# Quantco/tabmat

Measured on AMD Instinct MI355X. Metric: SplitMatrix.sandwich GFLOP/s + effective HBM GB/s, 10M×1k mixed, higher is better.
Workload: dtype f64; 1 GPU; SplitMatrix.sandwich: dense128 + csr512@5% + cats(256,96,32), 10000000 rows/GPU, p=1024, float64 (BASELINE configs[3]); rows_per_gpu=10000000, p=1024, launch=eager, collective=none

## Files before the change

tabmat_amd/csrc/syrk_co.hip:

```cpp
#include <algorithm>

#include "common.hpp"

namespace tmh {

constexpr int CO_RS = 12;
constexpr int CO_W = 128;
constexpr int CO_LDW = CO_W + 16;
constexpr int CO_CPI = 64;
constexpr int CO_ITEM_ROWS = CO_CPI * CO_RS;
constexpr int CO_T = 36;
constexpr int CO_NWAVES = 4;
constexpr int CO_THREADS = CO_NWAVES * 64;
constexpr int CO_CHUNK = CO_RS * CO_LDW;
constexpr size_t CO_LDS = sizeof(double) * (size_t)(2 * CO_CHUNK + 2 * CO_RS) + 32 + sizeof(double) * CO_W;
constexpr size_t CO_LDS_TV = CO_LDS + sizeof(double) * 2 * CO_RS;

typedef double co_acc_t __attribute__((ext_vector_type(4)));
typedef double co_vec2 __attribute__((ext_vector_type(2)));

constexpr int co_tri_row(int t) {
    int r = 0;
    while ((r + 1) * (r + 2) / 2 <= t) ++r;
    return r;
// ... 151 lines not shown
            for (int b = 0; b < 8; ++b) xa[b] = dv0 * xb0[b];
            cs0 += xa[2 * WID];
            cs1 += xa[2 * WID + 1];
            if constexpr (TV) {
                cv0 = __builtin_fma(vv0, xb0[2 * WID], cv0);
                cv1 = __builtin_fma(vv0, xb0[2 * WID + 1], cv1);
            }
            co_mfma_set<WID, 0>(xa, xb0, acc);
            __syncthreads();
            if (pending) { idNext = *slot; pending = false; }
            id_c = id_c1;
            id_c1 = id_c2;
            buf ^= 1;
        }
        double *dst = part + (int64_t)blockIdx.x * (CO_T * 256);
#pragma unroll
        for (int s = 0; s < 9; ++s) {
            const int t = WID + s * CO_NWAVES;
#pragma unroll
            for (int r = 0; r < 4; ++r)
                dst[t * 256 + ((lane >> 4) + 4 * r) * 16 + (lane & 15)] = acc[s][r];
        }
        cs0 += __shfl_xor(cs0, 16, 64);
        cs0 += __shfl_xor(cs0, 32, 64);
        cs1 += __shfl_xor(cs1, 16, 64);
        cs1 += __shfl_xor(cs1, 32, 64);
        if (lane < 16) {
            double *cd = cpart + (int64_t)blockIdx.x * CO_W;
            cd[32 * WID + 2 * lane] = cs0;
            cd[32 * WID + 2 * lane + 1] = cs1;
        }
        if constexpr (TV) {
            cv0 += __shfl_xor(cv0, 16, 64);
            cv0 += __shfl_xor(cv0, 32, 64);
            cv1 += __shfl_xor(cv1, 16, 64);
            cv1 += __shfl_xor(cv1, 32, 64);
            if (lane < 16) {
                double *vd = vpart + (int64_t)blockIdx.x * CO_W;
                vd[32 * WID + 2 * lane] = cv0;
                vd[32 * WID + 2 * lane + 1] = cv1;
            }
        }
    };
    if (wave == 0) run(std::integral_constant<int, 0>{});
    else if (wave == 1) run(std::integral_constant<int, 1>{});
    else if (wave == 2) run(std::integral_constant<int, 2>{});
    else run(std::integral_constant<int, 3>{});
    if (tid == 0) wg_log_end(log, t_begin, WG_SYRK_CO);
}

__global__ __launch_bounds__(1024) void syrk_co_finish_kernel(const double *__restrict__ part,
                                                              int nblk, int n_cols,
                                                              double *__restrict__ out, int64_t ldo,
                                                              const unsigned *__restrict__ only_if) {
    if (only_if != nullptr && *only_if == 0) return;
    __shared__ double red[16][64];
    const int e = blockIdx.y * 64 + threadIdx.x, s = threadIdx.y, t = blockIdx.x;
    double a = 0.0;
    for (int b = s; b < nblk; b += 16) a += part[((int64_t)b * CO_T + t) * 256 + e];
    red[s][threadIdx.x] = a;
    __syncthreads();
    if (s == 0) {
        double v = 0.0;
#pragma unroll
        for (int w = 0; w < 16; w += 4)
            v += (red[w][threadIdx.x] + red[w + 1][threadIdx.x]) +
                 (red[w + 2][threadIdx.x] + red[w + 3][threadIdx.x]);
        int bi = 0;
        while ((bi + 1) * (bi + 2) / 2 <= t) ++bi;
        const int bj = t - bi * (bi + 1) / 2;
        const int ci = co_actual_col(16 * bi + (e >> 4)), cj = co_actual_col(16 * bj + (e & 15));
        if (ci < n_cols && cj < n_cols && (bi != bj || (e >> 4) >= (e & 15))) {
            out[(int64_t)ci * ldo + cj] = v;
            if (ci != cj) out[(int64_t)cj * ldo + ci] = v;
        }
    }
}

__global__ __launch_bounds__(CO_W) void syrk_co_colsum_kernel(const double *__restrict__ cpart,
                                                              int nblk, int n_cols,
                                                              double *__restrict__ colsum,
                                                              const unsigned *__restrict__ only_if) {
    if (only_if != nullptr && *only_if == 0u) return;
    const int c = threadIdx.x;
    double a = 0.0;
    for (int b = 0; b < nblk; ++b) a += cpart[(int64_t)b * CO_W + c];
    if (c < n_cols) colsum[c] = a;
}

size_t syrk_co_ws_bytes() {
    const size_t grid = (size_t)std::max<int64_t>(1, tune("co_grid", 3 * NUM_CU));
    return 256 + sizeof(double) * grid * (CO_T * 256 + 2 * CO_W);
}

static int run_syrk_co_impl(const double *X, int64_t ldx, int64_t n, int64_t m, const double *d, double *out,
                            int64_t ldo, double *colsum, const unsigned *only_if, void *ws_given,
                            hipStream_t st, const double *center, const double *v, double *xtv) {
    TM_REQUIRE((v == nullptr) == (xtv == nullptr), "v and xtv go together");
    TM_REQUIRE(n >= 0 && m >= 0, "negative shape");
    TM_REQUIRE(m == 0 || syrk_co_ok(X, m),
               "the co-resident syrk takes a 16-byte aligned C-ordered block of <= 128 columns");
    if (m == 0) return TM_OK;
    if (n == 0) {
        TM_HIP(hipMemset2DAsync(out, sizeof(double) * (size_t)ldo, 0, sizeof(double) * (size_t)m, (size_t)m, st));
        if (colsum) TM_HIP(hipMemsetAsync(colsum, 0, sizeof(double) * (size_t)m, st));
        if (xtv) TM_HIP(hipMemsetAsync(xtv, 0, sizeof(double) * (size_t)m, st));
        return TM_OK;
    }
    const int64_t n_items64 = ceil_div(n, CO_ITEM_ROWS);
    TM_REQUIRE(n_items64 < (1ll << 31), "too many rows");
    const int n_items = (int)n_items64;
    const int grid = (int)std::min<int64_t>(n_items, tune("co_grid", 3 * NUM_CU));
    const size_t part_bytes = sizeof(double) * (size_t)grid * CO_T * 256;
    const size_t cpart_bytes = sizeof(double) * (size_t)grid * CO_W * (v ? 2 : 1);
    void *wsv = ws_given;
    if (wsv == nullptr) {
        int rc = get_workspace(256 + part_bytes + cpart_bytes, &wsv, st);
        if (rc) return rc;
    }
    unsigned *counter = reinterpret_cast<unsigned *>(wsv);
    double *part = reinterpret_cast<double *>(reinterpret_cast<char *>(wsv) + 256);
    double *cpart = part + (size_t)grid * CO_T * 256;
    double *vpart = v ? cpart + (size_t)grid * CO_W : nullptr;
    TM_HIP(hipMemsetAsync(counter, 0, 256, st));
    auto kern = v ? ((m & 1) ? (center ? &syrk_co_kernel<true, true, true> : &syrk_co_kernel<false, true, true>)
                             : (center ? &syrk_co_kernel<true, false, true> : &syrk_co_kernel<false, false, true>))
                  : ((m & 1) ? (center ? &syrk_co_kernel<true, true> : &syrk_co_kernel<false, true>)
                             : (center ? &syrk_co_kernel<true, false> : &syrk_co_kernel<false, false>));
    const size_t lds = v ? CO_LDS_TV : CO_LDS;
    TM_HIP(hipFuncSetAttribute(reinterpret_cast<const void *>(kern),
                               hipFuncAttributeMaxDynamicSharedMemorySize, (int)lds));
    prof_begin(st);
    hipLaunchKernelGGL(kern, dim3((unsigned)grid), dim3(CO_THREADS), lds, st, X, n, ldx,
                       (int)m, d, n_items, counter, part, cpart, wg_log_ptr(), only_if, center, v, vpart);
    prof_end(st);
    TM_LAUNCH_CHECK();
    hipLaunchKernelGGL(syrk_co_finish_kernel, dim3(CO_T, 4), dim3(64, 16), 0, st, part, grid, (int)m,
                       out, ldo, only_if);
    TM_LAUNCH_CHECK();
    if (colsum) {
        hipLaunchKernelGGL(syrk_co_colsum_kernel, dim3(1), dim3(CO_W), 0, st, cpart, grid, (int)m,
                           colsum, only_if);
        TM_LAUNCH_CHECK();
    }
    if (xtv) {
        hipLaunchKernelGGL(syrk_co_colsum_kernel, dim3(1), dim3(CO_W), 0, st, vpart, grid, (int)m,
                           xtv, only_if);
        TM_LAUNCH_CHECK();
    }
    return TM_OK;
}

int run_syrk_co(const double *X, int64_t n, int64_t m, const double *d, double *out, double *colsum,
                hipStream_t st, const double *center, const double *v, double *xtv) {
    return run_syrk_co_impl(X, m, n, m, d, out, m, colsum, nullptr, nullptr, st, center, v, xtv);
}

int run_syrk_co_flagged(const double *X, int64_t ldx, int64_t n, int64_t m, const double *d, double *out,
                        int64_t ldo, double *colsum, const unsigned *flag, void *ws, hipStream_t st,
                        const double *center, const double *v, double *xtv) {
    return run_syrk_co_impl(X, ldx, n, m, d, out, ldo, colsum, flag, ws, st, center, v, xtv);
}

}

using namespace tmh;

extern "C" {

int tm_dense_sandwich_co_f64(const double *X, int64_t n, int64_t m, const double *d, double *out,
                             double *colsum, void *stream) {
    return run_syrk_co(X, n, m, d, out, colsum, as_stream(stream));
}

int tm_dense_sandwich_co_centered_f64(const double *X, int64_t n, int64_t m, const double *d, const double *center,
                                      double *out, double *colsum, void *stream) {
    return run_syrk_co(X, n, m, d, out, colsum, as_stream(stream), center);
}

int tm_dense_sandwich_co_xtv_f64(const double *X, int64_t n, int64_t m, const double *d, const double *v,
                                 double *out, double *colsum, double *xtv, void *stream) {
    TM_REQUIRE(v != nullptr && xtv != nullptr, "v and xtv are required");
    return run_syrk_co(X, n, m, d, out, colsum, as_stream(stream), nullptr, v, xtv);
}

int tm_dense_sandwich_co_centered_xtv_f64(const double *X, int64_t n, int64_t m, const double *d, const double *v,
                                          const double *center, double *out, double *colsum, double *xtv,
                                          void *stream) {
    TM_REQUIRE(v != nullptr && xtv != nullptr, "v and xtv are required");
    return run_syrk_co(X, n, m, d, out, colsum, as_stream(stream), center, v, xtv);
}

}
```

tabmat_amd/csrc/syrk_i8.hip:

```cpp
#include <algorithm>
#include <cmath>

#include "common.hpp"

#if defined(I8_NO_SB)
#define I8_SB
#else
#define I8_SB __builtin_amdgcn_sched_barrier(0)
#endif
#if defined(I8_TRACE)
#define I8_STAMP(k)                                                                                     \
    do {                                                                                                \
        if (blockIdx.x == 0 && lane == 0 && trace_it >= 8 && trace_it < 12)                             \
            trace_buf[((trace_it - 8) * 4 + wave) * 8 + (k)] = __builtin_readcyclecounter();            \
    } while (0)
#else
#define I8_STAMP(k)
#endif
namespace tmh {

constexpr int I8_W = 128;
constexpr int I8_T = 36;
constexpr int I8_ND = 5;
constexpr int I8_WLO = 2;
constexpr int I8_NC = 2 * (I8_ND - 1) - I8_WLO + 1;
constexpr int I8_FBITS = 38;
constexpr int I8_RS = 64;
constexpr int I8_HS = 32;
constexpr int I8_WAVES = 4;
constexpr int I8_THREADS = I8_WAVES * 64;
constexpr int I8_PSTR = 64;
constexpr int I8_PLANE = I8_W * I8_PSTR;
constexpr int I8_PLANES = I8_ND * I8_PLANE;
constexpr int I8_RAWSTR = 1024 + 32;
constexpr int I8_RAWBUF = I8_HS * I8_RAWSTR;
#ifndef I8_DMA_AUX
#define I8_DMA_AUX 0
#endif
#ifndef I8_CPI_N
#define I8_CPI_N 32
#endif
constexpr int I8_CPI = I8_CPI_N;
constexpr int I8_ITEM_ROWS = I8_CPI * I8_RS;
constexpr size_t I8_LDS = (size_t)I8_PLANES + 3 * (size_t)I8_RAWBUF + 3 * I8_HS * sizeof(double) + 16;
static_assert(I8_LDS <= 160 * 1024, "planes + the ring of 3 half chunks fill the CU's LDS");

typedef int i8_v4 __attribute__((ext_vector_type(4)));

struct I8Info {
    unsigned dmax_bits_hi;
    unsigned dmax_bits_lo;
    unsigned flag;
    unsigned pad;
};

constexpr int i8_pair_find(int idx, bool want_s) {
    int k = 0;
    for (int w = I8_WLO; w <= 2 * (I8_ND - 1); ++w)
        for (int s = 0; s < I8_ND; ++s) {
            const int t = w - s;
            if (t < 0 || t >= I8_ND) continue;
            if (k == idx) return want_s ? s : t;
            ++k;
        }
    return -1;
}
constexpr int i8_pair_s(int idx) { return i8_pair_find(idx, true); }
constexpr int i8_pair_t(int idx) { return i8_pair_find(idx, false); }
constexpr int i8_count_pairs() {
    int k = 0;
    while (i8_pair_find(k, true) >= 0) ++k;
    return k;
}
constexpr int I8_NP = i8_count_pairs();
static_assert(I8_NP == 22, "the pair groups of the chunk loop are laid out for 22 pairs");

template <int WID>
struct I8Tiles {
    static constexpr int NB = 5;
    static constexpr int block(int l) {
        constexpr int B[4][5] = {{0, 1, 2, 3, 4}, {0, 1, 5, 6, 7}, {2, 3, 5, 6, 7}, {3, 4, 5, 6, 7}};
        return B[WID][l];
    }
    static constexpr int local(int b) {
        for (int l = 0; l < NB; ++l)
            if (block(l) == b) return l;
        return 0;
    }
    static constexpr int bi(int q) {
        constexpr int T[4][9] = {{1, 2, 3, 4, 2, 3, 4, 3, 4}, {5, 6, 7, 5, 6, 7, 6, 0, 1},
                                 {5, 6, 7, 5, 6, 7, 7, 2, 3}, {5, 6, 7, 4, 7, 4, 5, 6, 7}};
        return T[WID][q];
    }
    static constexpr int bj(int q) {
        constexpr int T[4][9] = {{0, 0, 0, 0, 1, 1, 1, 2, 2}, {0, 0, 0, 1, 1, 1, 5, 0, 1},
                                 {2, 2, 2, 3, 3, 3, 5, 2, 3}, {4, 4, 4, 3, 6, 4, 5, 6, 7}};
        return T[WID][q];
    }
    static constexpr int tile(int q) { return bi(q) * (bi(q) + 1) / 2 + bj(q); }
};

#if defined(__HIP_DEVICE_COMPILE__)
typedef __amdgpu_buffer_rsrc_t i8_rsrc_t;
__device__ __forceinline__ i8_rsrc_t i8_rsrc(const void *base, int64_t bytes) {
    const unsigned nb = bytes <= 0 ? 0u : (bytes > 0xFFFFFFFFll ? 0xFFFFFFFFu : (unsigned)bytes);
    return __builtin_amdgcn_make_buffer_rsrc(const_cast<void *>(base), 0, (int)nb, 0x00020000);
}
__device__ __forceinline__ void i8_dma16(i8_rsrc_t rs, void *lds, int voff) {
    __builtin_amdgcn_raw_ptr_buffer_load_lds(rs, (__attribute__((address_space(3))) void *)lds, 16, voff, 0, 0, I8_DMA_AUX);
}
__device__ __forceinline__ void i8_lds_barrier() { asm volatile("s_waitcnt lgkmcnt(0)\n\ts_barrier" ::: "memory"); }
__device__ __forceinline__ unsigned i8_perm(unsigned hi, unsigned lo, unsigned sel) {
    return __builtin_amdgcn_perm(hi, lo, sel);
}
#else
struct i8_rsrc_t {};
inline i8_rsrc_t i8_rsrc(const void *, int64_t) { return {}; }
inline void i8_dma16(i8_rsrc_t, void *, int) {}
inline void i8_lds_barrier() {}
inline unsigned i8_perm(unsigned, unsigned, unsigned) { return 0; }
#endif

__global__ __launch_bounds__(256) void i8_screen_kernel(const double *__restrict__ d, int64_t n, I8Info *info) {
    double mx = 0.0;
    bool bad = false;
    const int64_t stride = (int64_t)gridDim.x * blockDim.x;
    int64_t i = (int64_t)blockIdx.x * blockDim.x + threadIdx.x;
    for (; i + 3 * stride < n; i += 4 * stride) {
        const double v0 = d[i], v1 = d[i + stride], v2 = d[i + 2 * stride], v3 = d[i + 3 * stride];
        bad |= !(v0 >= 0.0) || !(v0 <= 1.7e308) || !(v1 >= 0.0) || !(v1 <= 1.7e308) ||
               !(v2 >= 0.0) || !(v2 <= 1.7e308) || !(v3 >= 0.0) || !(v3 <= 1.7e308);
        mx = fmax(fmax(mx, fmax(v0, v1)), fmax(v2, v3));
    }
    for (; i < n; i += stride) {
        const double v = d[i];
        bad |= !(v >= 0.0) || !(v <= 1.7e308);
        mx = fmax(mx, v);
    }
    for (int off = 32; off > 0; off >>= 1) {
        mx = fmax(mx, __shfl_down(mx, off, 64));
        bad |= (bool)__shfl_down((int)bad, off, 64);
    }
    __shared__ double wmx[4];
    __shared__ int wbad[4];
    if ((threadIdx.x & 63) == 0) {
        wmx[threadIdx.x >> 6] = mx;
        wbad[threadIdx.x >> 6] = (int)bad;
    }
    __syncthreads();
    if (threadIdx.x == 0) {
        mx = fmax(fmax(wmx[0], wmx[1]), fmax(wmx[2], wmx[3]));
        if (wbad[0] | wbad[1] | wbad[2] | wbad[3]) atomicOr(&info->flag, 1u);
        atomicMax(reinterpret_cast<unsigned long long *>(info), (unsigned long long)__double_as_longlong(mx > 0.0 ? mx : 0.0));
    }
}

__global__ void i8_scale_kernel(const double *__restrict__ colmax, int m, int64_t n_rows, I8Info *info,
                                double *__restrict__ sigma, double *__restrict__ rscale, int *history) {
    const int i = threadIdx.x;
    if (history != nullptr && i == 0) {
        const int calls = history[1]++;
        if (history[0] >= 3 && (calls & 31) != 0) atomicOr(&info->flag, 4u);
    }
    if (i >= I8_W) return;
    const double dmax = __longlong_as_double(*reinterpret_cast<const long long *>(info));
    if (history != nullptr && i < m && n_rows > 0) {
        const double prev = reinterpret_cast<const double *>(history + 4)[i];
        const double bound = fmin(64.0, 134217728.0 / (double)n_rows);
        if (prev > 0.0 && !(colmax[i] * colmax[i] * dmax <= bound * prev)) atomicOr(&info->flag, 4u);
    }
    __syncthreads();
    double s = 1.0, r = 1.0;
    if (i < m) {
        const double big = colmax[i] * sqrt(dmax);
        if (big > 0.0 && info->flag == 0) {
            int e;
            frexp(big, &e);
            s = ldexp(1.0, I8_FBITS - e);
            r = ldexp(1.0, e - I8_FBITS);
        }
    }
    sigma[i] = s;
    rscale[i] = r;
}

template <bool CSUM, bool CEN, bool TV = false>
__global__ __launch_bounds__(I8_THREADS) __attribute__((amdgpu_waves_per_eu(1, 1)))
void syrk_i8_kernel(const double *__restrict__ X, int64_t ldx, int64_t n, int64_t m, const double *__restrict__ d,
                    const double *__restrict__ sigma, const I8Info *__restrict__ info, int n_items,
                    unsigned *__restrict__ counter, double *__restrict__ part, double *__restrict__ colsum,
                    const double *__restrict__ center, const double *__restrict__ v = nullptr,
                    double *__restrict__ xtv = nullptr) {
    if (info->flag != 0) return;
    __shared__ __attribute__((aligned(16))) unsigned char planes[I8_PLANES];
    __shared__ __attribute__((aligned(16))) unsigned char raw[3 * I8_RAWBUF];
    __shared__ double dl[3 * I8_HS];
    __shared__ double vl[TV ? 3 * I8_HS : 1];
    __shared__ unsigned slot_mem[4];
    unsigned *slot = slot_mem;
#if defined(I8_TRACE)
    unsigned long long *trace_buf = reinterpret_cast<unsigned long long *>(reinterpret_cast<char *>(counter) - 256 + 2560);
    int trace_it = 0;
#endif

    const int tid = threadIdx.x;
    const int lane = tid & 63;
    const int wave = __builtin_amdgcn_readfirstlane(tid >> 6);
    const int cl = lane & 15, rq = lane >> 4;

    unsigned idL = blockIdx.x;
    int hL = 0;
    unsigned idNext;
    if (tid == 0) *slot = gridDim.x + atomicAdd(counter, 1u);
    __syncthreads();
    idNext = __builtin_amdgcn_readfirstlane(*slot);
    bool pending = false;

    using C0 = std::integral_constant<int, 0>;
    using C1 = std::integral_constant<int, 1>;
    double dreg = 0.0, vreg = 0.0;
    const int dma_voff = lane * 2 < m ? lane * 16 : 0x7ffffff0;
    auto issue_half = [&](int rb) -> unsigned {
        const unsigned id = idL;
        const int64_t tb = (int64_t)id * I8_ITEM_ROWS + (int64_t)hL * I8_HS;
        const int64_t left = min((n - tb) * ldx * 8, (int64_t)I8_HS * ldx * 8);
        const uint64_t xb = (uint64_t)(uintptr_t)(X + tb * ldx);
        const unsigned xlo = __builtin_amdgcn_readfirstlane((unsigned)xb);
        const unsigned xhi = __builtin_amdgcn_readfirstlane((unsigned)(xb >> 32));
        const unsigned nbytes = __builtin_amdgcn_readfirstlane(
            left <= 0 ? 0u : (left > 0xFFFFFFFFll ? 0xFFFFFFFFu : (unsigned)left));
        const i8_rsrc_t rs = i8_rsrc(reinterpret_cast<const void *>((uintptr_t)(((uint64_t)xhi << 32) | xlo)), nbytes);
        if (wave == 0 && lane < I8_HS) dreg = tb + lane < n ? d[tb + lane] : 0.0;
        if constexpr (TV) {
            if (wave == 0 && lane < I8_HS) vreg = tb + lane < n ? v[tb + lane] : 0.0;
        }
#if !defined(I8_ABLATE_NO_DMA)
#pragma unroll
        for (int j = 0; j < 8; ++j)
            i8_dma16(rs, raw + rb * I8_RAWBUF + (8 * wave + j) * I8_RAWSTR, (int)((8 * wave + j) * ldx * 8) + dma_voff);
#endif
        if (++hL == 2 * I8_CPI) {
            hL = 0;
            idL = idNext;
            if (tid == 0) *slot = gridDim.x + atomicAdd(counter, 1u);
            pending = true;
        }
        return id;
    };
    auto publish_d = [&](int rb) {
        if (wave == 0 && lane < I8_HS) dl[rb * I8_HS + lane] = sqrt(dreg);
        if constexpr (TV) {
            if (wave == 0 && lane < I8_HS) vl[rb * I8_HS + lane] = vreg;
        }
    };

    const double sg0 = sigma[32 * wave + cl], sg1 = sigma[32 * wave + 16 + cl];
    double cen0 = 0.0, cen1 = 0.0;
    if constexpr (CEN) {
        cen0 = 32 * wave + cl < m ? center[32 * wave + cl] : 0.0;
        cen1 = 32 * wave + 16 + cl < m ? center[32 * wave + 16 + cl] : 0.0;
    }
    double cs0 = 0.0, cs1 = 0.0;
    double cv0 = 0.0, cv1 = 0.0;
    const double MAGIC = 6755399441055744.0 + 551911719040.0;
    const unsigned raw_lds = (unsigned)(uintptr_t)(__attribute__((address_space(3))) unsigned char *)raw;
    const unsigned planes_lds = (unsigned)(uintptr_t)(__attribute__((address_space(3))) unsigned char *)planes;
    struct Quad { double x[4]; };
    auto quad_issue = [&](int rb, auto cb_c, auto qq_c) -> Quad {
        constexpr int cb = decltype(cb_c)::value, qq = decltype(qq_c)::value;
        Quad q;
#if defined(I8_ABLATE_NO_CONVERT) || defined(I8_ABLATE_DMA_ONLY)
        q.x[0] = q.x[1] = q.x[2] = q.x[3] = 0.0;
        return q;
#endif
        const int col = 32 * wave + 16 * cb + cl;
        const int row0 = 4 * (rq + 4 * qq);
        const unsigned ra = raw_lds + (unsigned)(rb * I8_RAWBUF + row0 * I8_RAWSTR + col * 8);
#if defined(__HIP_DEVICE_COMPILE__)
        asm volatile("ds_read_b64 %0, %4\n\tds_read_b64 %1, %4 offset:1056\n\tds_read_b64 %2, %4 offset:2112\n\t"
                     "ds_read_b64 %3, %4 offset:3168"
                     : "=&v"(q.x[0]), "=&v"(q.x[1]), "=&v"(q.x[2]), "=&v"(q.x[3])
                     : "v"(ra)
                     : "memory");
#else
        (void)ra;
        q.x[0] = q.x[1] = q.x[2] = q.x[3] = 0.0;
#endif
        static_assert(I8_RAWSTR == 1056, "the ds_read offsets above are multiples of the raw row stride");
        return q;
    };
    auto quad_wait = [&](Quad &q) {
#if defined(__HIP_DEVICE_COMPILE__) && !defined(I8_ABLATE_NO_CONVERT) && !defined(I8_ABLATE_DMA_ONLY)
        asm volatile("s_waitcnt lgkmcnt(0)" : "+v"(q.x[0]), "+v"(q.x[1]), "+v"(q.x[2]), "+v"(q.x[3])::"memory");
#endif
    };
    struct Conv {
        double dv[4];
        double vv[TV ? 4 : 1];
// ... 42 lines not shown
            c.g[1] = i8_perm(c.t[2], c.t[0], 0x07060302u) ^ 0x80808080u;
        } else if constexpr (k == 9) {
            c.g[2] = i8_perm(c.t[3], c.t[1], 0x05040100u) ^ 0x80808080u;
        } else if constexpr (k == 10) {
            c.g[3] = i8_perm(c.t[3], c.t[1], 0x07060302u) ^ 0x80808080u;
        } else if constexpr (k == 11) {
            c.h[0] = i8_perm(c.hi[1], c.hi[0], 0x05010400u);
            c.h[1] = i8_perm(c.hi[3], c.hi[2], 0x05010400u);
        } else if constexpr (k == 12) {
            c.g[4] = i8_perm(c.h[1], c.h[0], 0x05040100u) ^ 0x80808080u;
        } else if constexpr (k == 13) {
            const int col = 32 * wave + 16 * cb + cl;
            const unsigned pa =
                planes_lds + (unsigned)(col * I8_PSTR + (((2 * hh + qq) ^ ((cl >> 1) & 3)) << 4) + 4 * rq);
#if defined(__HIP_DEVICE_COMPILE__)
            asm volatile("ds_write_b32 %0, %1\n\tds_write_b32 %0, %2 offset:8192\n\tds_write_b32 %0, %3 offset:16384\n\t"
                         "ds_write_b32 %0, %4 offset:24576\n\tds_write_b32 %0, %5 offset:32768"
                         :
                         : "v"(pa), "v"(c.g[0]), "v"(c.g[1]), "v"(c.g[2]), "v"(c.g[3]), "v"(c.g[4])
                         : "memory");
#else
            (void)pa;
#endif
            static_assert(I8_PLANE == 8192 && I8_ND == 5, "the ds_write offsets above are the plane strides");
        }
    };
    constexpr int I8_CSTEPS = 14;
    constexpr int I8_CLAT = 3;
    auto quad_convert = [&](const Quad &q, int rb, int hh, auto cb_c, auto qq_c) {
        Conv c;
        static_for<I8_CSTEPS>([&](auto kc) { conv_step(kc, q, c, rb, hh, cb_c, qq_c); });
    };
    auto convert_quad = [&](int rb, int hh, auto cb_c, auto qq_c) {
        Quad q = quad_issue(rb, cb_c, qq_c);
        quad_wait(q);
        quad_convert(q, rb, hh, cb_c, qq_c);
    };
    auto convert_half = [&](int rb, int hh) {
        convert_quad(rb, hh, C0{}, C0{});
        convert_quad(rb, hh, C0{}, C1{});
        convert_quad(rb, hh, C1{}, C0{});
        convert_quad(rb, hh, C1{}, C1{});
    };

    const int foff = (lane & 15) * I8_PSTR + (((lane >> 4) ^ ((lane >> 1) & 3)) << 4);
    auto frag = [&](int b, int s) {
        return *reinterpret_cast<const i8_v4 *>(planes + s * I8_PLANE + b * 16 * I8_PSTR + foff);
    };

    auto run = [&](auto wid) {
        constexpr int WID = decltype(wid)::value;
        i8_v4 acc[9][I8_NC];
        double *dst = part + (int64_t)blockIdx.x * (I8_T * 256);
        auto flush = [&]() {
            asm volatile("s_nop 15\n\ts_nop 7" ::: "memory");
            unsigned lane_off = (unsigned)(((4 * (lane >> 4)) * 16 + (lane & 15)) * 8);
            asm volatile("" : "+v"(lane_off));
            char *const fb = reinterpret_cast<char *>(dst) + lane_off;
            static_for<9>([&](auto sc) {
                constexpr int s9 = decltype(sc)::value;
                constexpr int t = I8Tiles<WID>::tile(s9);
#pragma unroll
                for (int r = 0; r < 4; ++r) {
                    double v = (double)acc[s9][I8_NC - 1][r];
#pragma unroll
                    for (int c = I8_NC - 2; c >= 0; --c) v = v * 256.0 + (double)acc[s9][c][r];
                    atomicAdd(reinterpret_cast<double *>(fb + (t * 256 + r * 16) * 8), v);
                }
            });
        };

        unsigned id_c = issue_half(0);
        asm volatile("s_waitcnt vmcnt(8)" ::: "memory");
        publish_d(0);
        (void)issue_half(1);
        asm volatile("s_waitcnt vmcnt(8)" ::: "memory");
        publish_d(1);
        asm volatile("s_waitcnt vmcnt(0)" ::: "memory");
        i8_lds_barrier();
        if (pending) { idNext = __builtin_amdgcn_readfirstlane(*slot); pending = false; }
        convert_half(0, 0);
        convert_half(1, 1);
        i8_lds_barrier();
        unsigned id_c1 = issue_half(2);
        asm volatile("s_waitcnt vmcnt(8)" ::: "memory");
        publish_d(2);
        (void)issue_half(0);
        asm volatile("s_waitcnt vmcnt(8)" ::: "memory");
        publish_d(0);
        int sa = 2;

        while (id_c < (unsigned)n_items) {
#pragma unroll
          for (int t = 0; t < 9; ++t)
#pragma unroll
              for (int c = 0; c < I8_NC; ++c) {
                  acc[t][c] = i8_v4{0, 0, 0, 0};
                  asm volatile("" : "+a"(acc[t][c]));
              }
          for (int oc = 0; oc < I8_CPI; ++oc) {
            I8_STAMP(0);
            const int sb = sa == 2 ? 0 : sa + 1;
            const int sc = sb == 2 ? 0 : sb + 1;
            i8_lds_barrier();
            I8_STAMP(1);
            if (pending) { idNext = __builtin_amdgcn_readfirstlane(*slot); pending = false; }
            Quad qa = quad_issue(sa, C0{}, C0{});
            using TL = I8Tiles<WID>;
            i8_v4 F[TL::NB][I8_ND];
            auto mf = [&](auto lo_c, auto hi_c) {
                constexpr int LO = decltype(lo_c)::value, HI = decltype(hi_c)::value;
                static_for<HI - LO>([&](auto ic) {
                    constexpr int k = LO + decltype(ic)::value;
                    constexpr int idx = k / 9, q = k % 9;
                    constexpr int ps = i8_pair_s(idx), pt = i8_pair_t(idx);
#if defined(I8_ABLATE_DMA_ONLY)
                    return;
#endif
                    i8_v4 &cacc = acc[q][ps + pt - I8_WLO];
                    const i8_v4 fa = F[TL::local(TL::bi(q))][ps], fb = F[TL::local(TL::bj(q))][pt];
                    asm volatile("v_mfma_i32_16x16x64_i8 %0, %1, %2, %0" : "+a"(cacc) : "v"(fa), "v"(fb));
                });
            };
#define I8_MF(lo, hi) mf(std::integral_constant<int, lo>{}, std::integral_constant<int, hi>{})
            static_for<I8_ND>([&](auto oc_) {
                constexpr int order[I8_ND] = {0, 2, 1, 3, 4};
                constexpr int sd = order[decltype(oc_)::value];
#pragma unroll
                for (int b = 0; b < TL::NB; ++b) {
#if defined(I8_ABLATE_DMA_ONLY)
                    F[b][sd] = i8_v4{0, 0, 0, 0};
#else
                    F[b][sd] = frag(TL::block(b), sd);
#endif
                }
            });
            static_assert(i8_pair_s(0) == 0 && i8_pair_t(0) == 2 && i8_pair_s(2) == 2 && i8_pair_s(3) + i8_pair_t(3) == 3,
                          "the first three pairs are class 2");
            I8_MF(0, 27);
#if !defined(I8_NO_WEAVE)
            __builtin_amdgcn_sched_group_barrier(0x100, 10, 0);
            static_for<15>([&](auto) {
                __builtin_amdgcn_sched_group_barrier(0x008, 1, 0);
                __builtin_amdgcn_sched_group_barrier(0x100, 1, 0);
            });
            __builtin_amdgcn_sched_group_barrier(0x008, 12, 0);
#endif
            I8_SB;
            I8_STAMP(2);
            i8_lds_barrier();
            I8_STAMP(3);
            quad_wait(qa);
            const unsigned id_a = issue_half(sc);
// ... 13 lines not shown
#define I8_GROUP(lo, hi, q, rb, hh, cb, qq) \
    group(std::integral_constant<int, lo>{}, std::integral_constant<int, hi>{}, q, rb, hh, cb, qq)
            Quad qb = quad_issue(sa, C0{}, C1{});
            I8_GROUP(27, 49, qa, sa, 0, C0{}, C0{});
            quad_wait(qb);
            I8_SB;
            qa = quad_issue(sa, C1{}, C0{});
            I8_GROUP(49, 71, qb, sa, 0, C0{}, C1{});
            quad_wait(qa);
            I8_SB;
            qb = quad_issue(sa, C1{}, C1{});
            I8_GROUP(71, 93, qa, sa, 0, C1{}, C0{});
            quad_wait(qb);
            I8_SB;
            I8_GROUP(93, 114, qb, sa, 0, C1{}, C1{});
            I8_SB;
            I8_STAMP(4);
            asm volatile("s_waitcnt vmcnt(8)" ::: "memory");
            publish_d(sc);
            I8_STAMP(5);
            i8_lds_barrier();
            I8_STAMP(6);
            (void)issue_half(sa);
            qa = quad_issue(sb, C0{}, C0{});
            I8_MF(114, 120);
            quad_wait(qa);
            I8_SB;
            qb = quad_issue(sb, C0{}, C1{});
            I8_GROUP(120, 140, qa, sb, 1, C0{}, C0{});
            quad_wait(qb);
            I8_SB;
            qa = quad_issue(sb, C1{}, C0{});
            I8_GROUP(140, 160, qb, sb, 1, C0{}, C1{});
            quad_wait(qa);
            I8_SB;
            qb = quad_issue(sb, C1{}, C1{});
            I8_GROUP(160, 180, qa, sb, 1, C1{}, C0{});
            quad_wait(qb);
            I8_SB;
            I8_GROUP(180, 198, qb, sb, 1, C1{}, C1{});
            I8_SB;
#undef I8_MF
#undef I8_GROUP
            static_assert(I8_NP * 9 == 198, "the group bounds above");
            I8_STAMP(7);
            asm volatile("s_waitcnt vmcnt(8)" ::: "memory");
            publish_d(sa);
#if defined(I8_TRACE)
            ++trace_it;
#endif
            sa = sc;
            id_c = id_c1;
            id_c1 = id_a;
          }
          flush();
        }
    };
    if (wave == 0) run(std::integral_constant<int, 0>{});
    else if (wave == 1) run(std::integral_constant<int, 1>{});
    else if (wave == 2) run(std::integral_constant<int, 2>{});
    else run(std::integral_constant<int, 3>{});
    asm volatile("s_waitcnt vmcnt(0)" ::: "memory");
    if constexpr (CSUM) {
        cs0 += __shfl_xor(cs0, 16, 64);
        cs0 += __shfl_xor(cs0, 32, 64);
        cs1 += __shfl_xor(cs1, 16, 64);
        cs1 += __shfl_xor(cs1, 32, 64);
        if (lane < 16) {
            if (32 * wave + cl < m) atomicAdd(colsum + 32 * wave + cl, cs0);
            if (32 * wave + 16 + cl < m) atomicAdd(colsum + 32 * wave + 16 + cl, cs1);
        }
    }
    if constexpr (TV) {
        cv0 += __shfl_xor(cv0, 16, 64);
        cv0 += __shfl_xor(cv0, 32, 64);
        cv1 += __shfl_xor(cv1, 16, 64);
        cv1 += __shfl_xor(cv1, 32, 64);
        if (lane < 16) {
            if (32 * wave + cl < m) atomicAdd(xtv + 32 * wave + cl, cv0);
            if (32 * wave + 16 + cl < m) atomicAdd(xtv + 32 * wave + 16 + cl, cv1);
        }
    }
}

__global__ __launch_bounds__(1024) void syrk_i8_finish_kernel(const double *__restrict__ part, int nblk,
                                                              int n_cols, const double *__restrict__ rscale,
                                                              const I8Info *__restrict__ info,
                                                              double *__restrict__ out, int64_t ldo) {
    if (info->flag != 0) return;
#if defined(I8_TRACE)
    if (blockIdx.x == 0 && blockIdx.y == 0 && threadIdx.y == 0) {
        const unsigned long long *tb = reinterpret_cast<const unsigned long long *>(reinterpret_cast<const char *>(info) + 2560);
        for (int k = threadIdx.x; k < 128; k += 64) out[k] = (double)(tb[k] - tb[0]);
    }
    return;
#endif
    __shared__ double red[16][64];
    const int e = blockIdx.y * 64 + threadIdx.x, s = threadIdx.y, t = blockIdx.x;
    double a = 0.0;
    for (int b = s; b < nblk; b += 16) a += part[((int64_t)b * I8_T + t) * 256 + e];
    red[s][threadIdx.x] = a;
    __syncthreads();
    if (s == 0) {
        double v = 0.0;
#pragma unroll
        for (int w = 0; w < 16; w += 4)
            v += (red[w][threadIdx.x] + red[w + 1][threadIdx.x]) + (red[w + 2][threadIdx.x] + red[w + 3][threadIdx.x]);
        int bi = 0;
        while ((bi + 1) * (bi + 2) / 2 <= t) ++bi;
        const int bj = t - bi * (bi + 1) / 2;
        const int ci = 16 * bi + (e >> 4), cj = 16 * bj + (e & 15);
        if (ci < n_cols && cj < n_cols && (bi != bj || (e >> 4) >= (e & 15))) {
            v = v * 65536.0 * rscale[ci] * rscale[cj];
            static_assert(I8_WLO == 2, "65536 = 256^I8_WLO");
            out[(int64_t)ci * ldo + cj] = v;
            if (ci != cj) out[(int64_t)cj * ldo + ci] = v;
        }
    }
}

__global__ void i8_envelope_kernel(const double *__restrict__ out, int64_t ldo, const double *__restrict__ colmax,
                                   int m, int64_t n, I8Info *info, int *history) {
    const int j = threadIdx.x;
    __shared__ int miss;
    if (j == 0) miss = 0;
    __syncthreads();
    const bool live = info->flag == 0;
#if defined(I8_TRACE)
    return;
#endif
    if (j < m && live) {
        const double dmax = __longlong_as_double(*reinterpret_cast<const long long *>(info));
        const double big2 = colmax[j] * colmax[j] * dmax;
        const double bound = fmin(64.0, 134217728.0 / (double)n);
        if (!(big2 <= bound * out[(int64_t)j * ldo + j])) {
            atomicOr(&info->flag, 2u);
            miss = 1;
        }
    }
    __syncthreads();
    if (history != nullptr && j == 0 && live) history[0] = miss ? history[0] + 1 : 0;
}

__global__ void i8_record_diag_kernel(const double *__restrict__ out, int64_t ldo, int m, int *history) {
    const int j = threadIdx.x;
    if (j < I8_W) reinterpret_cast<double *>(history + 4)[j] = j < m ? out[(int64_t)j * ldo + j] : 0.0;
}

int run_syrk_co_flagged(const double *X, int64_t ldx, int64_t n, int64_t m, const double *d, double *out,
                        int64_t ldo, double *colsum, const unsigned *flag, void *ws, hipStream_t st,
                        const double *center, const double *v, double *xtv);
size_t syrk_co_ws_bytes();

int run_syrk_i8_panel(const double *X, int64_t ldx, int64_t n, int64_t m, const double *d, const double *colmax,
                      double *out, int64_t ldo, double *colsum, int *history, hipStream_t st, const double *center,
                      const double *v, double *xtv) {
    TM_REQUIRE((v == nullptr) == (xtv == nullptr), "v and xtv go together");
    TM_REQUIRE(v == nullptr || colsum == nullptr, "X' d and X' v are not built into one int8 kernel");
    TM_REQUIRE(n >= 0 && m >= 0, "negative shape");
    TM_REQUIRE(ldx >= m && ldo >= m, "row strides");
    TM_REQUIRE(m == 0 || syrk_co_ok(X, m), "the int8 syrk takes a 16-byte aligned C-ordered f64 block of <= 128 columns");
    if (m == 0) return TM_OK;
    if (n == 0) {
        TM_HIP(hipMemset2DAsync(out, sizeof(double) * (size_t)ldo, 0, sizeof(double) * (size_t)m, (size_t)m, st));
        if (colsum) TM_HIP(hipMemsetAsync(colsum, 0, sizeof(double) * (size_t)m, st));
        if (xtv) TM_HIP(hipMemsetAsync(xtv, 0, sizeof(double) * (size_t)m, st));
        return TM_OK;
    }
    if (colsum) TM_HIP(hipMemsetAsync(colsum, 0, sizeof(double) * (size_t)m, st));
    if (xtv) TM_HIP(hipMemsetAsync(xtv, 0, sizeof(double) * (size_t)m, st));
    const int64_t n_items64 = ceil_div(n, I8_ITEM_ROWS);
    TM_REQUIRE(n_items64 < (1ll << 31), "too many rows");
    const int n_items = (int)n_items64;
    const int grid = (int)std::max<int64_t>(1, std::min<int64_t>(n_items, tune("i8_grid", NUM_CU)));
    const size_t part_bytes = sizeof(double) * (size_t)grid * I8_T * 256;
    const size_t own_bytes = (4096 + part_bytes + 255) / 256 * 256;
    void *wsv = nullptr;
    int rc = get_workspace(own_bytes + syrk_co_ws_bytes(), &wsv, st);
    if (rc) return rc;
    char *wb = reinterpret_cast<char *>(wsv);
    I8Info *info = reinterpret_cast<I8Info *>(wb);
    unsigned *counter = reinterpret_cast<unsigned *>(wb + 256);
    double *sigma = reinterpret_cast<double *>(wb + 512);
    double *rscale = reinterpret_cast<double *>(wb + 512 + 1024);
    double *part = reinterpret_cast<double *>(wb + 4096);
    TM_HIP(hipMemsetAsync(wb, 0, 4096 + part_bytes, st));
    const int sgrid = (int)std::min<int64_t>(4 * NUM_CU, ceil_div(n, 1024));
    hipLaunchKernelGGL(i8_screen_kernel, dim3((unsigned)sgrid), dim3(256), 0, st, d, n, info);
    hipLaunchKernelGGL(i8_scale_kernel, dim3(1), dim3(I8_W), 0, st, colmax, (int)m, n, info, sigma, rscale, history);
    TM_LAUNCH_CHECK();
    prof_begin(st);
    auto go = [&](auto kern) {
        hipLaunchKernelGGL(kern, dim3((unsigned)grid), dim3(I8_THREADS), 0, st, X, ldx, n, m, d, sigma, info, n_items,
                           counter, part, colsum, center, v, xtv);
    };
    if (v) {
        if (center) go(syrk_i8_kernel<false, true, true>);
        else go(syrk_i8_kernel<false, false, true>);
    } else if (center) {
        if (colsum) go(syrk_i8_kernel<true, true>);
        else go(syrk_i8_kernel<false, true>);
    } else {
        if (colsum) go(syrk_i8_kernel<true, false>);
        else go(syrk_i8_kernel<false, false>);
    }
    prof_end(st);
    TM_LAUNCH_CHECK();
    hipLaunchKernelGGL(syrk_i8_finish_kernel, dim3(I8_T, 4), dim3(64, 16), 0, st, part, grid, (int)m, rscale, info,
                       out, ldo);
    hipLaunchKernelGGL(i8_envelope_kernel, dim3(1), dim3(I8_W), 0, st, out, ldo, colmax, (int)m, n, info, history);
    TM_LAUNCH_CHECK();
    prof_hold(true);
    rc = run_syrk_co_flagged(X, ldx, n, m, d, out, ldo, colsum, &info->flag, wb + own_bytes, st, center, v, xtv);
    prof_hold(false);
    if (rc == TM_OK && history != nullptr) {
        hipLaunchKernelGGL(i8_record_diag_kernel, dim3(1), dim3(I8_W), 0, st, out, ldo, (int)m, history);
        TM_LAUNCH_CHECK();
    }
    return rc;
}

int run_syrk_i8(const double *X, int64_t n, int64_t m, const double *d, const double *colmax, double *out,
                double *colsum, int *history, hipStream_t st, const double *center = nullptr,
                const double *v = nullptr, double *xtv = nullptr) {
    return run_syrk_i8_panel(X, m, n, m, d, colmax, out, m, colsum, history, st, center, v, xtv);
}

}

extern "C" {

int tm_dense_sandwich_i8_history_words(void) { return 4 + 2 * tmh::I8_W; }

int tm_dense_sandwich_i8_f64(const double *X, int64_t n, int64_t m, const double *d, const double *colmax,
                             double *out, void *stream) {
    return tmh::run_syrk_i8(X, n, m, d, colmax, out, nullptr, nullptr, tmh::as_stream(stream));
}

int tm_dense_sandwich_i8_xtd_f64(const double *X, int64_t n, int64_t m, const double *d, const double *colmax,
                                 double *out, double *colsum, void *stream) {
    return tmh::run_syrk_i8(X, n, m, d, colmax, out, colsum, nullptr, tmh::as_stream(stream));
}

int tm_dense_sandwich_i8_hist_f64(const double *X, int64_t n, int64_t m, const double *d, const double *colmax,
                                  double *out, double *colsum, int32_t *history, void *stream) {
    return tmh::run_syrk_i8(X, n, m, d, colmax, out, colsum, history, tmh::as_stream(stream));
}

int tm_dense_sandwich_i8_centered_f64(const double *X, int64_t n, int64_t m, const double *d, const double *colmax,
                                      const double *center, double *out, double *colsum, int32_t *history,
                                      void *stream) {
    return tmh::run_syrk_i8(X, n, m, d, colmax, out, colsum, history, tmh::as_stream(stream), center);
}

int tm_dense_sandwich_i8_xtv_f64(const double *X, int64_t n, int64_t m, const double *d, const double *v,
                                 const double *colmax, double *out, double *xtv, int32_t *history, void *stream) {
    TM_REQUIRE(v != nullptr && xtv != nullptr, "v and xtv are required");
    return tmh::run_syrk_i8(X, n, m, d, colmax, out, nullptr, history, tmh::as_stream(stream), nullptr, v, xtv);
}

int tm_dense_sandwich_i8_centered_xtv_f64(const double *X, int64_t n, int64_t m, const double *d, const double *v,
                                          const double *colmax, const double *center, double *out, double *xtv,
                                          int32_t *history, void *stream) {
    TM_REQUIRE(v != nullptr && xtv != nullptr, "v and xtv are required");
    return tmh::run_syrk_i8(X, n, m, d, colmax, out, nullptr, history, tmh::as_stream(stream), center, v, xtv);
}

}
```

Before: 1044 GB/s.

## Fuse i8 syrk prep and envelope kernels, balance items per workgroup adaptively

The separate screen/scale kernels become one prep kernel that uses a last-block ticket, and the envelope check and diagonal recording move into the finish kernels. Together these drop several tiny launches. Chunks-per-item is now picked at runtime so work splits evenly across the grid. The first flush of each workgroup stores its partials directly instead of using atomics, so the large memset of the partial buffer goes away. In exchange, grid-wide ticket synchronisation and extra bookkeeping are added to the finish and prep paths.

After: 1033 GB/s. 1.1% lower.

```diff
diff --git a/tabmat_amd/csrc/syrk_co.hip b/tabmat_amd/csrc/syrk_co.hip
--- a/tabmat_amd/csrc/syrk_co.hip
+++ b/tabmat_amd/csrc/syrk_co.hip
@@ -227,7 +227,8 @@
 __global__ __launch_bounds__(1024) void syrk_co_finish_kernel(const double *__restrict__ part,
                                                               int nblk, int n_cols,
                                                               double *__restrict__ out, int64_t ldo,
-                                                              const unsigned *__restrict__ only_if) {
+                                                              const unsigned *__restrict__ only_if,
+                                                              double *__restrict__ diag_out) {
     if (only_if != nullptr && *only_if == 0) return;
     __shared__ double red[16][64];
     const int e = blockIdx.y * 64 + threadIdx.x, s = threadIdx.y, t = blockIdx.x;
@@ -249,6 +250,7 @@
             out[(int64_t)ci * ldo + cj] = v;
             if (ci != cj) out[(int64_t)cj * ldo + ci] = v;
         }
+        if (diag_out != nullptr && ci == cj && ci < CO_W) diag_out[ci] = ci < n_cols ? v : 0.0;
     }
 }
 
@@ -270,7 +272,8 @@
 
 static int run_syrk_co_impl(const double *X, int64_t ldx, int64_t n, int64_t m, const double *d, double *out,
                             int64_t ldo, double *colsum, const unsigned *only_if, void *ws_given,
-                            hipStream_t st, const double *center, const double *v, double *xtv) {
+                            hipStream_t st, const double *center, const double *v, double *xtv,
+                            double *diag_out = nullptr) {
     TM_REQUIRE((v == nullptr) == (xtv == nullptr), "v and xtv go together");
     TM_REQUIRE(n >= 0 && m >= 0, "negative shape");
     TM_REQUIRE(m == 0 || syrk_co_ok(X, m),
@@ -311,7 +314,7 @@
     prof_end(st);
     TM_LAUNCH_CHECK();
     hipLaunchKernelGGL(syrk_co_finish_kernel, dim3(CO_T, 4), dim3(64, 16), 0, st, part, grid, (int)m,
-                       out, ldo, only_if);
+                       out, ldo, only_if, diag_out);
     TM_LAUNCH_CHECK();
     if (colsum) {
         hipLaunchKernelGGL(syrk_co_colsum_kernel, dim3(1), dim3(CO_W), 0, st, cpart, grid, (int)m,
@@ -333,8 +336,8 @@
 
 int run_syrk_co_flagged(const double *X, int64_t ldx, int64_t n, int64_t m, const double *d, double *out,
                         int64_t ldo, double *colsum, const unsigned *flag, void *ws, hipStream_t st,
-                        const double *center, const double *v, double *xtv) {
-    return run_syrk_co_impl(X, ldx, n, m, d, out, ldo, colsum, flag, ws, st, center, v, xtv);
+                        const double *center, const double *v, double *xtv, double *diag_out) {
+    return run_syrk_co_impl(X, ldx, n, m, d, out, ldo, colsum, flag, ws, st, center, v, xtv, diag_out);
 }
 
 }
diff --git a/tabmat_amd/csrc/syrk_i8.hip b/tabmat_amd/csrc/syrk_i8.hip
--- a/tabmat_amd/csrc/syrk_i8.hip
+++ b/tabmat_amd/csrc/syrk_i8.hip
@@ -38,10 +38,12 @@
 #define I8_DMA_AUX 0
 #endif
 #ifndef I8_CPI_N
-#define I8_CPI_N 32
-#endif
-constexpr int I8_CPI = I8_CPI_N;
-constexpr int I8_ITEM_ROWS = I8_CPI * I8_RS;
+#define I8_CPI_N 0
+#endif
+constexpr int I8_CPI_MAX = 384;
+static_assert(5ll * I8_W * I8_W * ((long long)I8_CPI_MAX * I8_RS) < (1ll << 31),
+              "a class holds <= 5 pairs of products |b_s b_t| <= 128 * 128: exact in int32 over a whole item");
+static_assert(I8_CPI_N >= 0 && I8_CPI_N <= I8_CPI_MAX, "I8_CPI_N");
 constexpr size_t I8_LDS = (size_t)I8_PLANES + 3 * (size_t)I8_RAWBUF + 3 * I8_HS * sizeof(double) + 16;
 static_assert(I8_LDS <= 160 * 1024, "planes + the ring of 3 half chunks fill the CU's LDS");
 
@@ -121,7 +123,18 @@
 inline unsigned i8_perm(unsigned, unsigned, unsigned) { return 0; }
 #endif
 
-__global__ __launch_bounds__(256) void i8_screen_kernel(const double *__restrict__ d, int64_t n, I8Info *info) {
+__device__ __forceinline__ unsigned i8_peek(const unsigned *p) {
+    return __hip_atomic_load(p, __ATOMIC_RELAXED, __HIP_MEMORY_SCOPE_AGENT);
+}
+__device__ __forceinline__ double i8_peek_dmax(const I8Info *info) {
+    return __longlong_as_double((long long)__hip_atomic_load(reinterpret_cast<const unsigned long long *>(info),
+                                                             __ATOMIC_RELAXED, __HIP_MEMORY_SCOPE_AGENT));
+}
+
+__global__ __launch_bounds__(256) void i8_prep_kernel(const double *__restrict__ d, int64_t n,
+                                                      const double *__restrict__ colmax, int m, I8Info *info,
+                                                      unsigned *ticket, double *__restrict__ sigma,
+                                                      double *__restrict__ rscale, int *history) {
     double mx = 0.0;
     bool bad = false;
     const int64_t stride = (int64_t)gridDim.x * blockDim.x;
@@ -143,6 +156,7 @@
     }
     __shared__ double wmx[4];
     __shared__ int wbad[4];
+    __shared__ int last;
     if ((threadIdx.x & 63) == 0) {
         wmx[threadIdx.x >> 6] = mx;
         wbad[threadIdx.x >> 6] = (int)bad;
@@ -152,42 +166,44 @@
         mx = fmax(fmax(wmx[0], wmx[1]), fmax(wmx[2], wmx[3]));
         if (wbad[0] | wbad[1] | wbad[2] | wbad[3]) atomicOr(&info->flag, 1u);
         atomicMax(reinterpret_cast<unsigned long long *>(info), (unsigned long long)__double_as_longlong(mx > 0.0 ? mx : 0.0));
-    }
-}
-
-__global__ void i8_scale_kernel(const double *__restrict__ colmax, int m, int64_t n_rows, I8Info *info,
-                                double *__restrict__ sigma, double *__restrict__ rscale, int *history) {
-    const int i = threadIdx.x;
-    if (history != nullptr && i == 0) {
+        __threadfence();
+        last = atomicAdd(ticket, 1u) == gridDim.x - 1;
+    }
+    __syncthreads();
+    if (!last) return;
+    __threadfence();
+    const int c = threadIdx.x;
+    if (history != nullptr && c == 0) {
         const int calls = history[1]++;
         if (history[0] >= 3 && (calls & 31) != 0) atomicOr(&info->flag, 4u);
     }
-    if (i >= I8_W) return;
-    const double dmax = __longlong_as_double(*reinterpret_cast<const long long *>(info));
-    if (history != nullptr && i < m && n_rows > 0) {
-        const double prev = reinterpret_cast<const double *>(history + 4)[i];
-        const double bound = fmin(64.0, 134217728.0 / (double)n_rows);
-        if (prev > 0.0 && !(colmax[i] * colmax[i] * dmax <= bound * prev)) atomicOr(&info->flag, 4u);
-    }
+    const double dmax = i8_peek_dmax(info);
+    if (history != nullptr && c < m && n > 0) {
+        const double prev = reinterpret_cast<const double *>(history + 4)[c];
+        const double bound = fmin(64.0, 134217728.0 / (double)n);
+        if (prev > 0.0 && !(colmax[c] * colmax[c] * dmax <= bound * prev)) atomicOr(&info->flag, 4u);
+    }
+    __threadfence();
     __syncthreads();
+    if (c >= I8_W) return;
     double s = 1.0, r = 1.0;
-    if (i < m) {
-        const double big = colmax[i] * sqrt(dmax);
-        if (big > 0.0 && info->flag == 0) {
+    if (c < m) {
+        const double big = colmax[c] * sqrt(dmax);
+        if (big > 0.0 && i8_peek(&info->flag) == 0) {
             int e;
             frexp(big, &e);
             s = ldexp(1.0, I8_FBITS - e);
             r = ldexp(1.0, e - I8_FBITS);
         }
     }
-    sigma[i] = s;
-    rscale[i] = r;
+    sigma[c] = s;
+    rscale[c] = r;
 }
 
 template <bool CSUM, bool CEN, bool TV = false>
 __global__ __launch_bounds__(I8_THREADS) __attribute__((amdgpu_waves_per_eu(1, 1)))
 void syrk_i8_kernel(const double *__restrict__ X, int64_t ldx, int64_t n, int64_t m, const double *__restrict__ d,
-                    const double *__restrict__ sigma, const I8Info *__restrict__ info, int n_items,
+                    const double *__restrict__ sigma, const I8Info *__restrict__ info, int n_items, int cpi,
                     unsigned *__restrict__ counter, double *__restrict__ part, double *__restrict__ colsum,
                     const double *__restrict__ center, const double *__restrict__ v = nullptr,
                     double *__restrict__ xtv = nullptr) {
@@ -208,12 +224,17 @@
     const int wave = __builtin_amdgcn_readfirstlane(tid >> 6);
     const int cl = lane & 15, rq = lane >> 4;
 
+    const int64_t item_rows = (int64_t)cpi * I8_RS;
     unsigned idL = blockIdx.x;
     int hL = 0;
     unsigned idNext;
+#if defined(I8_STATIC_ITEMS)
+    idNext = blockIdx.x + gridDim.x;
+#else
     if (tid == 0) *slot = gridDim.x + atomicAdd(counter, 1u);
     __syncthreads();
     idNext = __builtin_amdgcn_readfirstlane(*slot);
+#endif
     bool pending = false;
 
     using C0 = std::integral_constant<int, 0>;
@@ -222,7 +243,7 @@
     const int dma_voff = lane * 2 < m ? lane * 16 : 0x7ffffff0;
     auto issue_half = [&](int rb) -> unsigned {
         const unsigned id = idL;
-        const int64_t tb = (int64_t)id * I8_ITEM_ROWS + (int64_t)hL * I8_HS;
+        const int64_t tb = (int64_t)id * item_rows + (int64_t)hL * I8_HS;
         const int64_t left = min((n - tb) * ldx * 8, (int64_t)I8_HS * ldx * 8);
         const uint64_t xb = (uint64_t)(uintptr_t)(X + tb * ldx);
         const unsigned xlo = __builtin_amdgcn_readfirstlane((unsigned)xb);
@@ -239,11 +260,15 @@
         for (int j = 0; j < 8; ++j)
             i8_dma16(rs, raw + rb * I8_RAWBUF + (8 * wave + j) * I8_RAWSTR, (int)((8 * wave + j) * ldx * 8) + dma_voff);
 #endif
-        if (++hL == 2 * I8_CPI) {
+        if (++hL == 2 * cpi) {
             hL = 0;
             idL = idNext;
+#if defined(I8_STATIC_ITEMS)
+            idNext += gridDim.x;
+#else
             if (tid == 0) *slot = gridDim.x + atomicAdd(counter, 1u);
             pending = true;
+#endif
         }
         return id;
     };
@@ -392,7 +417,8 @@
         constexpr int WID = decltype(wid)::value;
         i8_v4 acc[9][I8_NC];
         double *dst = part + (int64_t)blockIdx.x * (I8_T * 256);
-        auto flush = [&]() {
+        auto flush = [&](auto store_c) {
+            constexpr bool STORE = decltype(store_c)::value;
             asm volatile("s_nop 15\n\ts_nop 7" ::: "memory");
             unsigned lane_off = (unsigned)(((4 * (lane >> 4)) * 16 + (lane & 15)) * 8);
             asm volatile("" : "+v"(lane_off));
@@ -405,7 +431,9 @@
                     double v = (double)acc[s9][I8_NC - 1][r];
 #pragma unroll
                     for (int c = I8_NC - 2; c >= 0; --c) v = v * 256.0 + (double)acc[s9][c][r];
-                    atomicAdd(reinterpret_cast<double *>(fb + (t * 256 + r * 16) * 8), v);
+                    double *const pd = reinterpret_cast<double *>(fb + (t * 256 + r * 16) * 8);
+                    if constexpr (STORE) *pd = v;
+                    else atomicAdd(pd, v);
                 }
             });
         };
@@ -430,6 +458,7 @@
         publish_d(0);
         int sa = 2;
 
+        bool first = true;
         while (id_c < (unsigned)n_items) {
 #pragma unroll
           for (int t = 0; t < 9; ++t)
@@ -438,7 +467,8 @@
                   acc[t][c] = i8_v4{0, 0, 0, 0};
                   asm volatile("" : "+a"(acc[t][c]));
               }
-          for (int oc = 0; oc < I8_CPI; ++oc) {
+          int oc = 0;
+          do {
             I8_STAMP(0);
             const int sb = sa == 2 ? 0 : sa + 1;
             const int sc = sb == 2 ? 0 : sb + 1;
@@ -558,8 +588,10 @@
             sa = sc;
             id_c = id_c1;
             id_c1 = id_a;
-          }
-          flush();
+          } while (++oc < cpi);
+          if (first) flush(std::true_type{});
+          else flush(std::false_type{});
+          first = false;
         }
     };
     if (wave == 0) run(std::integral_constant<int, 0>{});
@@ -591,9 +623,10 @@
 
 __global__ __launch_bounds__(1024) void syrk_i8_finish_kernel(const double *__restrict__ part, int nblk,
                                                               int n_cols, const double *__restrict__ rscale,
-                                                              const I8Info *__restrict__ info,
-                                                              double *__restrict__ out, int64_t ldo) {
-    if (info->flag != 0) return;
+                                                              I8Info *info, double *__restrict__ out, int64_t ldo,
+                                                              const double *__restrict__ colmax, int64_t n,
+                                                              unsigned *ticket, int *history) {
+    if ((i8_peek(&info->flag) & ~2u) != 0) return;
 #if defined(I8_TRACE)
     if (blockIdx.x == 0 && blockIdx.y == 0 && threadIdx.y == 0) {
         const unsigned long long *tb = reinterpret_cast<const unsigned long long *>(reinterpret_cast<const char *>(info) + 2560);
@@ -622,41 +655,54 @@
             out[(int64_t)ci * ldo + cj] = v;
             if (ci != cj) out[(int64_t)cj * ldo + ci] = v;
         }
-    }
-}
-
-__global__ void i8_envelope_kernel(const double *__restrict__ out, int64_t ldo, const double *__restrict__ colmax,
-                                   int m, int64_t n, I8Info *info, int *history) {
-    const int j = threadIdx.x;
-    __shared__ int miss;
-    if (j == 0) miss = 0;
+        if (ci == cj) {
+            if (ci < n_cols) {
+                const double big2 = colmax[ci] * colmax[ci] * i8_peek_dmax(info);
+                const double bound = fmin(64.0, 134217728.0 / (double)n);
+                if (!(big2 <= bound * v)) {
+                    atomicOr(&info->flag, 2u);
+                    __threadfence();
+                }
+            }
+            if (history != nullptr) reinterpret_cast<double *>(history + 4)[ci] = ci < n_cols ? v : 0.0;
+        }
+    }
     __syncthreads();
-    const bool live = info->flag == 0;
-#if defined(I8_TRACE)
-    return;
-#endif
-    if (j < m && live) {
-        const double dmax = __longlong_as_double(*reinterpret_cast<const long long *>(info));
-        const double big2 = colmax[j] * colmax[j] * dmax;
-        const double bound = fmin(64.0, 134217728.0 / (double)n);
-        if (!(big2 <= bound * out[(int64_t)j * ldo + j])) {
-            atomicOr(&info->flag, 2u);
-            miss = 1;
-        }
-    }
-    __syncthreads();
-    if (history != nullptr && j == 0 && live) history[0] = miss ? history[0] + 1 : 0;
-}
-
-__global__ void i8_record_diag_kernel(const double *__restrict__ out, int64_t ldo, int m, int *history) {
-    const int j = threadIdx.x;
-    if (j < I8_W) reinterpret_cast<double *>(history + 4)[j] = j < m ? out[(int64_t)j * ldo + j] : 0.0;
+    if (threadIdx.x == 0 && threadIdx.y == 0 && atomicAdd(ticket, 1u) == gridDim.x * gridDim.y - 1) {
+        __threadfence();
+        if (history != nullptr) history[0] = (i8_peek(&info->flag) & 2u) ? history[0] + 1 : 0;
+    }
 }
 
 int run_syrk_co_flagged(const double *X, int64_t ldx, int64_t n, int64_t m, const double *d, double *out,
                         int64_t ldo, double *colsum, const unsigned *flag, void *ws, hipStream_t st,
-                        const double *center, const double *v, double *xtv);
+                        const double *center, const double *v, double *xtv, double *diag_out);
 size_t syrk_co_ws_bytes();
+
+#ifndef I8_CPI_TARGET_N
+#define I8_CPI_TARGET_N 32
+#endif
+struct I8Geom {
+    int cpi, grid;
+    int64_t n_items;
+};
+static I8Geom i8_geometry(int64_t n) {
+    const int64_t n_chunks = ceil_div(n, I8_RS);
+    const int64_t G = std::max<int64_t>(1, tune("i8_grid", NUM_CU));
+    int64_t cpi = tune("i8_cpi", I8_CPI_N);
+    if (cpi <= 0) {
+        const int64_t per_wg = ceil_div(n_chunks, G);
+        const int64_t target = std::max<int64_t>(1, std::min<int64_t>(tune("i8_cpi_target", I8_CPI_TARGET_N), I8_CPI_MAX));
+        const int64_t rounds = ceil_div(per_wg, target);
+        cpi = std::max<int64_t>(tune("i8_cmin", 2), ceil_div(n_chunks, G * rounds));
+    }
+    cpi = std::max<int64_t>(1, std::min<int64_t>(cpi, I8_CPI_MAX));
+    I8Geom g;
+    g.cpi = (int)cpi;
+    g.n_items = ceil_div(n_chunks, cpi);
+    g.grid = (int)std::min<int64_t>(G, g.n_items);
+    return g;
+}
 
 int run_syrk_i8_panel(const double *X, int64_t ldx, int64_t n, int64_t m, const double *d, const double *colmax,
                       double *out, int64_t ldo, double *colsum, int *history, hipStream_t st, const double *center,
@@ -675,10 +721,9 @@
     }
     if (colsum) TM_HIP(hipMemsetAsync(colsum, 0, sizeof(double) * (size_t)m, st));
     if (xtv) TM_HIP(hipMemsetAsync(xtv, 0, sizeof(double) * (size_t)m, st));
-    const int64_t n_items64 = ceil_div(n, I8_ITEM_ROWS);
-    TM_REQUIRE(n_items64 < (1ll << 31), "too many rows");
-    const int n_items = (int)n_items64;
-    const int grid = (int)std::max<int64_t>(1, std::min<int64_t>(n_items, tune("i8_grid", NUM_CU)));
+    const I8Geom geo = i8_geometry(n);
+    TM_REQUIRE(geo.n_items < (1ll << 31), "too many rows");
+    const int n_items = (int)geo.n_items, cpi = geo.cpi, grid = geo.grid;
     const size_t part_bytes = sizeof(double) * (size_t)grid * I8_T * 256;
     const size_t own_bytes = (4096 + part_bytes + 255) / 256 * 256;
     void *wsv = nullptr;
@@ -687,18 +732,20 @@
     char *wb = reinterpret_cast<char *>(wsv);
     I8Info *info = reinterpret_cast<I8Info *>(wb);
     unsigned *counter = reinterpret_cast<unsigned *>(wb + 256);
+    unsigned *prep_ticket = reinterpret_cast<unsigned *>(wb + 320);
+    unsigned *finish_ticket = reinterpret_cast<unsigned *>(wb + 384);
     double *sigma = reinterpret_cast<double *>(wb + 512);
     double *rscale = reinterpret_cast<double *>(wb + 512 + 1024);
     double *part = reinterpret_cast<double *>(wb + 4096);
-    TM_HIP(hipMemsetAsync(wb, 0, 4096 + part_bytes, st));
+    TM_HIP(hipMemsetAsync(wb, 0, 4096, st));
     const int sgrid = (int)std::min<int64_t>(4 * NUM_CU, ceil_div(n, 1024));
-    hipLaunchKernelGGL(i8_screen_kernel, dim3((unsigned)sgrid), dim3(256), 0, st, d, n, info);
-    hipLaunchKernelGGL(i8_scale_kernel, dim3(1), dim3(I8_W), 0, st, colmax, (int)m, n, info, sigma, rscale, history);
+    hipLaunchKernelGGL(i8_prep_kernel, dim3((unsigned)sgrid), dim3(256), 0, st, d, n, colmax, (int)m, info, prep_ticket,
+                       sigma, rscale, history);
     TM_LAUNCH_CHECK();
     prof_begin(st);
     auto go = [&](auto kern) {
         hipLaunchKernelGGL(kern, dim3((unsigned)grid), dim3(I8_THREADS), 0, st, X, ldx, n, m, d, sigma, info, n_items,
-                           counter, part, colsum, center, v, xtv);
+                           cpi, counter, part, colsum, center, v, xtv);
     };
     if (v) {
         if (center) go(syrk_i8_kernel<false, true, true>);
@@ -713,16 +760,12 @@
     prof_end(st);
     TM_LAUNCH_CHECK();
     hipLaunchKernelGGL(syrk_i8_finish_kernel, dim3(I8_T, 4), dim3(64, 16), 0, st, part, grid, (int)m, rscale, info,
-                       out, ldo);
-    hipLaunchKernelGGL(i8_envelope_kernel, dim3(1), dim3(I8_W), 0, st, out, ldo, colmax, (int)m, n, info, history);
+                       out, ldo, colmax, n, finish_ticket, history);
     TM_LAUNCH_CHECK();
     prof_hold(true);
-    rc = run_syrk_co_flagged(X, ldx, n, m, d, out, ldo, colsum, &info->flag, wb + own_bytes, st, center, v, xtv);
+    rc = run_syrk_co_flagged(X, ldx, n, m, d, out, ldo, colsum, &info->flag, wb + own_bytes, st, center, v, xtv,
+                             history ? reinterpret_cast<double *>(history + 4) : nullptr);
     prof_hold(false);
-    if (rc == TM_OK && history != nullptr) {
-        hipLaunchKernelGGL(i8_record_diag_kernel, dim3(1), dim3(I8_W), 0, st, out, ldo, (int)m, history);
-        TM_LAUNCH_CHECK();
-    }
     return rc;
 }
 
```
